# TuringLang/AdvancedHMC.jl

Measured on NVIDIA B200. Metric: leapfrog-steps*dims/sec, higher is better.
Workload: dtype f64

## Files before the change

### advancedhmc.jl_b200/__init__.py

```python
from . import _lib
from ._lib import (FLAG_ASYNC, FLAG_COMPAT_BREAK_ALL, FLAG_EXACT_CHECKS, FLAG_HOST_BUFFERS, FLAG_NO_REFRESH,
                   FLAG_NUTS_CLASSIC, FLAG_NUTS_SLICE_TS, FLAG_NUTS_STRICT,
                   STATUS_NONFINITE, AhmcError, InvalidArgument)
from .core import *
from .core import get_context
```

### advancedhmc.jl_b200/_lib.py

```python
from __future__ import annotations

import ctypes as C
import os

HERE = os.path.dirname(os.path.abspath(__file__))
LIB_PATH = os.environ.get("AHMC_B200_LIB", os.path.join(HERE, "libahmc_b200.so"))

OK, ERR_INVALID, ERR_CUDA, ERR_UNSUPPORTED, ERR_NOMEM, ERR_CALLBACK = 0, -1, -2, -3, -4, -5
METRIC_UNIT, METRIC_DIAG, METRIC_DENSE = 0, 1, 2
MODEL_STD_NORMAL, MODEL_DIAG_GAUSS, MODEL_DENSE_GAUSS, MODEL_FUNNEL, MODEL_CALLBACK, MODEL_USER = 0, 1, 2, 3, 4, 5
FLAG_HOST_BUFFERS, FLAG_COMPAT_BREAK_ALL, FLAG_ASYNC, FLAG_EXACT_CHECKS, FLAG_NO_REFRESH = 1, 2, 4, 8, 16
FLAG_NUTS_SLICE_TS, FLAG_NUTS_CLASSIC, FLAG_NUTS_STRICT = 32, 64, 128
STATUS_NONFINITE = 1

_dp = C.POINTER(C.c_double)
_vp = C.c_void_p


class Metric(C.Structure):
    _fields_ = [("kind", C.c_int32), ("Minv", _vp), ("chain_stride", C.c_int64), ("cholU", _vp)]


class PhasePoint(C.Structure):
    _fields_ = [("theta", _vp), ("r", _vp), ("lp_value", _vp), ("lp_gradient", _vp), ("lk_value", _vp),
                ("lk_gradient", _vp), ("ld", C.c_int64)]


class Stats(C.Structure):
    _fields_ = [("n_steps", _vp), ("is_accept", _vp), ("acceptance_rate", _vp), ("log_density", _vp),
                ("hamiltonian_energy", _vp), ("hamiltonian_energy_error", _vp),
                ("max_hamiltonian_energy_error", _vp), ("tree_depth", _vp), ("numerical_error", _vp)]


class Rng(C.Structure):
    _fields_ = [("seed", C.c_uint64), ("offset", C.c_uint64), ("normal_tape", _vp), ("exp_tape", _vp),
                ("exp_stride", C.c_int64), ("dir_tape", _vp), ("dir_stride", C.c_int64),
                ("partial_refresh_alpha", C.c_double), ("temper_alpha", C.c_double)]


class AdaptCfg(C.Structure):
    _fields_ = [("n_adapts", C.c_int32), ("init_buffer", C.c_int32), ("term_buffer", C.c_int32), ("window_size", C.c_int32),
                ("delta", C.c_double), ("gamma", C.c_double), ("t0", C.c_double), ("kappa", C.c_double),
                ("adapt_metric", C.c_int32), ("n_min", C.c_int32), ("eps_chain", _vp), ("Minv_chain", _vp),
                ("eps_trace", _vp)]


class PooledCfg(C.Structure):
    _fields_ = [("n_adapts", C.c_int32), ("init_buffer", C.c_int32), ("term_buffer", C.c_int32), ("window_size", C.c_int32),
                ("delta", C.c_double), ("gamma", C.c_double), ("t0", C.c_double), ("kappa", C.c_double), ("eps0", C.c_double),
                ("adapt_metric", C.c_int32), ("n_min", C.c_int32)]


LOGP_GRAD_FN = C.CFUNCTYPE(C.c_int, _vp, _vp, _vp, _vp, C.c_int32, C.c_int64, C.c_int64, _vp)

PROTOTYPES = {
    "ahmc_version": (C.c_char_p, []),
    "ahmc_create": (C.c_int, [C.POINTER(_vp), C.c_int32, _vp]),
    "ahmc_destroy": (C.c_int, [_vp]),
    "ahmc_last_error": (C.c_char_p, [_vp]),
    "ahmc_synchronize": (C.c_int, [_vp]),
    "ahmc_stream": (_vp, [_vp]),
    "ahmc_launch_count": (C.c_int64, [_vp]),
    "ahmc_last_transport": (C.c_char_p, [_vp]),
    "ahmc_model_create": (C.c_int, [_vp, C.c_int32, C.c_int32, _dp, _dp, C.c_double, C.POINTER(_vp)]),
    "ahmc_model_create_callback": (C.c_int, [_vp, C.c_int32, LOGP_GRAD_FN, _vp, C.POINTER(_vp)]),
    "ahmc_model_create_user": (C.c_int, [_vp, C.c_int32, C.c_char_p, _dp, C.c_int32, C.c_double, C.POINTER(_vp)]),
    "ahmc_user_source_check": (C.c_int, [C.c_char_p, C.c_int32, C.c_int32, C.c_int32, C.c_char_p, C.c_int64]),
    "ahmc_model_destroy": (C.c_int, [_vp, _vp]),
    "ahmc_phasepoint_f64": (C.c_int, [_vp, _vp, C.POINTER(Metric), C.c_int32, C.c_int64, C.POINTER(PhasePoint),
                                      C.c_uint32]),
    "ahmc_leapfrog_f64": (C.c_int, [_vp, _vp, C.POINTER(Metric), C.c_int32, C.c_int64, C.c_double, _vp, C.c_int32,
                                    C.c_double, C.POINTER(PhasePoint), C.POINTER(PhasePoint), _vp, _vp, C.c_uint32]),
    "ahmc_leapfrog_trajectory_f64": (C.c_int, [_vp, _vp, C.POINTER(Metric), C.c_int32, C.c_int64, C.c_double, _vp,
                                               C.c_int32, C.c_double, C.POINTER(PhasePoint), C.POINTER(PhasePoint),
                                               C.c_int64, _vp, C.c_uint32]),
    "ahmc_hmc_multinomial_transition_f64": (C.c_int, [_vp, _vp, C.POINTER(Metric), C.c_int32, C.c_int64, C.c_double, _vp,
                                                      C.c_int32, C.c_int32, C.POINTER(Rng), C.POINTER(PhasePoint),
                                                      C.POINTER(PhasePoint), C.POINTER(Stats), C.c_uint32]),
    "ahmc_rand_momentum_f64": (C.c_int, [_vp, C.POINTER(Metric), C.c_int32, C.c_int64, C.POINTER(Rng), _vp,
                                         C.c_int64, C.c_uint32]),
    "ahmc_hmc_transition_f64": (C.c_int, [_vp, _vp, C.POINTER(Metric), C.c_int32, C.c_int64, C.c_double, _vp,
                                          C.c_int32, C.POINTER(Rng), C.POINTER(PhasePoint), C.POINTER(PhasePoint),
                                          C.POINTER(Stats), C.c_uint32]),
    "ahmc_nuts_transition_f64": (C.c_int, [_vp, _vp, C.POINTER(Metric), C.c_int32, C.c_int64, C.c_double, _vp,
                                           C.c_int32, C.c_double, C.POINTER(Rng), C.POINTER(PhasePoint),
                                           C.POINTER(PhasePoint), C.POINTER(Stats), C.c_uint32]),
    "ahmc_hmc_sample_f64": (C.c_int, [_vp, _vp, C.POINTER(Metric), C.c_int32, C.c_int64, C.c_double, _vp, C.c_int32,
                                      C.c_int32, C.POINTER(Rng), C.POINTER(PhasePoint), C.POINTER(PhasePoint), _vp,
                                      C.POINTER(Stats), C.c_uint32]),
    "ahmc_nuts_sample_f64": (C.c_int, [_vp, _vp, C.POINTER(Metric), C.c_int32, C.c_int64, C.c_double, _vp, C.c_int32,
                                       C.c_double, C.c_int32, C.POINTER(Rng), C.POINTER(PhasePoint),
                                       C.POINTER(PhasePoint), _vp, C.POINTER(Stats), C.c_uint32]),
    "ahmc_nuts_adapt_sample_f64": (C.c_int, [_vp, _vp, C.POINTER(Metric), C.c_int32, C.c_int64, C.c_int32, C.c_double,
                                             C.c_int32, C.POINTER(AdaptCfg), C.POINTER(Rng), C.POINTER(PhasePoint),
                                             C.POINTER(PhasePoint), _vp, C.POINTER(Stats), C.c_uint32]),
# ... 46 lines not shown
```

### advancedhmc.jl_b200/csrc/ahmc_leapfrog.cu

```cuda
#ifndef __CUDACC_RTC__
#include <cstdlib>
#endif
#include "ahmc_kernels.cuh"
#include "ahmc_traj.cuh"

namespace ahmc {

bool pick_layout(int D, int* G, int* E) {
    if (D < 1) return false;
    if (D <= 4) { *G = 4; *E = 1; return true; }
    if (D <= 8) { *G = 8; *E = 1; return true; }
    if (D <= 16) { *G = 16; *E = 1; return true; }
    if (D <= 32) { *G = 32; *E = 1; return true; }
    if (D <= 64) { *G = 32; *E = 2; return true; }
    if (D <= 128) { *G = 32; *E = 4; return true; }
    if (D <= 256) { *G = 32; *E = 8; return true; }
    if (D <= 512) { *G = 32; *E = 16; return true; }
    return false;
}

template <int G, int E, bool CONTIG = false>
struct StepIO {
    static constexpr bool kContig = CONTIG;
    const LeapfrogArgs& a;
    long long chain;
    int l;
    __device__ __forceinline__ bool has_g() const { return a.g_in != nullptr; }
    __device__ __forceinline__ void init(double (&th)[E], double (&r)[E], double (&g)[E]) const {
        vload_nc<G, E>(th, a.th_in + a.ld_in * chain, l, a.D);
        vload_nc<G, E>(r, a.r_in + a.ld_in * chain, l, a.D);
        if (a.g_in) vload_nc<G, E>(g, a.g_in + a.ld_in * chain, l, a.D);
    }
    __device__ __forceinline__ void init_c(double (&th)[E], double (&r)[E], double (&g)[E]) const {
        cload<E>(th, a.th_in + a.ld_in * chain, l, a.D);
        cload<E>(r, a.r_in + a.ld_in * chain, l, a.D);
        cload<E>(g, (a.g_in ? a.g_in : a.th_in) + a.ld_in * chain, l, a.D);
    }
    __device__ __forceinline__ void scalars(double lp, double lk, bool fin, int steps) const {
        if (l == 0) {
            a.lp_out[chain] = lp;
            a.lk_out[chain] = lk;
            if (a.status) a.status[chain] = fin ? 0u : AHMC_STATUS_NONFINITE;
            if (a.steps_done) a.steps_done[chain] = steps;
            if (!fin && a.min_break) atomicMin(a.min_break, steps);
        }
    }
    __device__ __forceinline__ void done(const double (&th)[E], const double (&r)[E], const double (&g)[E],
                                         const double (&dr)[E], double lp, double lk, bool fin, int steps) const {
        vstore<G, E>(a.th_out + a.ld_out * chain, th, l, a.D);
        vstore<G, E>(a.r_out + a.ld_out * chain, r, l, a.D);
        vstore<G, E>(a.g_out + a.ld_out * chain, g, l, a.D);
        if (a.dr_out) vstore<G, E>(a.dr_out + a.ld_out * chain, dr, l, a.D);
        scalars(lp, lk, fin, steps);
    }
    __device__ __forceinline__ void done_c(const double (&th)[E], const double (&r)[E], const double (&g)[E],
                                           const double (&dr)[E], double lp, double lk, bool fin, int steps) const {
        cstore<E>(a.th_out + a.ld_out * chain, th, l, a.D);
        cstore<E>(a.r_out + a.ld_out * chain, r, l, a.D);
        cstore<E>(a.g_out + a.ld_out * chain, g, l, a.D);
        if (a.dr_out) cstore<E>(a.dr_out + a.ld_out * chain, dr, l, a.D);
        scalars(lp, lk, fin, steps);
    }
};

template <int MODEL, int METRIC, int E>
constexpr int min_blocks_per_sm() {
    return (FastCapable<MODEL, METRIC>::value && E <= 4) ? 7 : 1;
}
template <int MODEL, int METRIC, int E>
constexpr int min_blocks_hmc() {
    return (FastCapable<MODEL, METRIC>::value && E <= 4) ? 7 : ((METRIC != AHMC_METRIC_DENSE && MODEL != AHMC_MODEL_DENSE_GAUSS && E <= 4) ? 4 : 1);
}
template <int MODEL, int METRIC, int E>
constexpr int min_blocks_lf() {
    return (MODEL == AHMC_MODEL_FUNNEL && METRIC != AHMC_METRIC_DENSE && E <= 4) ? 7 : min_blocks_per_sm<MODEL, METRIC, E>();
}

template <int MODEL, int METRIC, int G, int E, bool CONTIG = false>
__global__ void __launch_bounds__(kBlockThreads, min_blocks_lf<MODEL, METRIC, E>()) leapfrog_kernel(const LeapfrogArgs a) {
    extern __shared__ double smem[];
    const int l = threadIdx.x % G;
    const int grp_in_block = threadIdx.x / G;
    const long long chain0 = (long long)blockIdx.x * (kBlockThreads / G) + grp_in_block;
    const long long chain = chain0 < a.N ? chain0 : a.N - 1;
    const bool valid = chain0 < a.N && (!a.only_mask || a.only_mask[chain] != 0);
    double* xs = smem + (size_t)grp_in_block * slab_vectors<MODEL>() * a.D;
    double eps = a.eps_chain ? __ldg(a.eps_chain + chain) : a.eps;
    eps = a.fwd ? eps : -eps;
    StepIO<G, E, CONTIG> io{a, chain, l};
    run_trajectory<MODEL, METRIC, G, E>(a.model, a.metric, a.D, chain, valid, l, xs, eps, a.n_steps, a.temper_alpha,
                                        a.flags, io);
}

template <int METRIC, int G, int E>
struct HmcIO {
    const HmcArgs& h;
    long long chain;
    int l;
    const double* src_th;
    const double* src_g;
    long long stat_idx;
    double H0, lp0, lk0, ex;
    double r0[E];

    static constexpr bool kContig = false;
    __device__ __forceinline__ bool has_g() const { return true; }
    __device__ __forceinline__ void init(double (&th)[E], double (&r)[E], double (&g)[E]) const {
        vload_nc<G, E>(th, src_th, l, h.lf.D);
        vload_nc<G, E>(g, src_g, l, h.lf.D);
#pragma unroll
        for (int e = 0; e < E; ++e) r[e] = r0[e];
    }
    __device__ __forceinline__ void done(const double (&th)[E], const double (&r)[E], const double (&g)[E],
                                         const double (&dr)[E], double lp, double lk, bool fin, int steps) const {
        const LeapfrogArgs& a = h.lf;
        const double H1 = -(lp + lk);
        const bool accept = H1 < H0 + ex;
        double alpha = exp(H0 - H1);
        alpha = (alpha != alpha) ? alpha : (alpha < 1.0 ? alpha : 1.0);
        double* tho = a.th_out + a.ld_out * chain;
        double* ro = a.r_out + a.ld_out * chain;
        double* go = a.g_out + a.ld_out * chain;
        double* dro = h.draws ? h.draws + stat_idx * a.D : nullptr;
        double lpn, lkn;
        if (accept) {
            double nr[E];
#pragma unroll
            for (int e = 0; e < E; ++e) nr[e] = -r[e];
            vstore<G, E>(tho, th, l, a.D);
            vstore<G, E>(ro, nr, l, a.D);
            vstore<G, E>(go, g, l, a.D);
            if (dro) vstore<G, E>(dro, th, l, a.D);
            lpn = lp;
            lkn = lk;
        } else {
            double t0[E], g0[E], nr[E];
            vload_nc<G, E>(t0, src_th, l, a.D);
            vload_nc<G, E>(g0, src_g, l, a.D);
#pragma unroll
            for (int e = 0; e < E; ++e) nr[e] = -r0[e];
            vstore<G, E>(tho, t0, l, a.D);
            vstore<G, E>(ro, nr, l, a.D);
            vstore<G, E>(go, g0, l, a.D);
            if (dro) vstore<G, E>(dro, t0, l, a.D);
            lpn = lp0;
            lkn = lk0;
        }
        if (l == 0) {
            const double H = -(lpn + lkn);
            a.lp_out[chain] = lpn;
            a.lk_out[chain] = lkn;
            if (a.status) a.status[chain] = fin ? 0u : AHMC_STATUS_NONFINITE;
            if (a.steps_done) a.steps_done[chain] = steps;
            const StatsDev& st = h.st;
            if (st.n_steps) st.n_steps[stat_idx] = a.n_steps;
            if (st.is_accept) st.is_accept[stat_idx] = accept ? 1 : 0;
            if (st.acceptance_rate) st.acceptance_rate[stat_idx] = alpha;
            if (st.log_density) st.log_density[stat_idx] = lpn;
            if (st.hamiltonian_energy) st.hamiltonian_energy[stat_idx] = H;
            if (st.hamiltonian_energy_error) st.hamiltonian_energy_error[stat_idx] = H - H0;
            if (st.numerical_error) st.numerical_error[stat_idx] = finite_d(H1) ? 0 : 1;
        }
        (void)dr;
    }
};

template <int MODEL, int METRIC, int G, int E>
__global__ void __launch_bounds__(kBlockThreads, min_blocks_hmc<MODEL, METRIC, E>()) hmc_kernel(const HmcArgs h) {
    extern __shared__ double smem[];
    const LeapfrogArgs& a = h.lf;
    const int l = threadIdx.x % G;
    const int grp_in_block = threadIdx.x / G;
    const long long chain0 = (long long)blockIdx.x * (kBlockThreads / G) + grp_in_block;
    const bool valid = chain0 < a.N;
// ... 214 lines not shown
    const double lp = a.cb_lp ? a.cb_lp[chain] : 0.0;
    bool fin = true;
#pragma unroll
    for (int e = 0; e < E; ++e) fin = fin && finite_d(g[e]) && finite_d(dr[e]);
    fin = Grp<G>::all(fin) && finite_d(lp) && finite_d(lk);
    if (active) {
        if (!a.no_kick) vstore<G, E>(a.r + a.ld * chain, r, l, D);
        if (a.cb_grad) vstore<G, E>(a.g + a.ld * chain, g, l, D);
        if (a.dr) vstore<G, E>(a.dr + a.ld * chain, dr, l, D);
        if (l == 0) {
            if (a.cb_lp) a.lp[chain] = map_nonfinite(lp);
            a.lk[chain] = map_nonfinite(lk);
            if (!a.no_kick) {
                if (a.steps_done) a.steps_done[chain] = a.step_index;
                if (!fin) {
                    a.status[chain] = AHMC_STATUS_NONFINITE;
                    if (a.any_nonfinite) *a.any_nonfinite = 1;
                }
            }
        }
    }
}

template <int G, int E>
__global__ void __launch_bounds__(kBlockThreads) mh_select_kernel(const MhArgs a) {
    const int l = threadIdx.x % G;
    const long long chain0 = (long long)blockIdx.x * (kBlockThreads / G) + threadIdx.x / G;
    if (chain0 >= a.N) return;
    const long long chain = chain0;
    const int D = a.D;
    const double lp0 = map_nonfinite(a.lp0[chain]), lk0 = a.lk0[chain];
    const double lp1 = a.lp[chain], lk1 = a.lk[chain];
    const double H0 = -(lp0 + lk0), H1 = -(lp1 + lk1);
    const double ex = a.rng.exp_tape ? a.rng.exp_tape[chain] : philox_exp(a.rng.seed, a.rng.offset, chain, 0);
    const bool accept = H1 < H0 + ex;
    double alpha = exp(H0 - H1);
    alpha = (alpha != alpha) ? alpha : (alpha < 1.0 ? alpha : 1.0);
    double t[E];
    if (accept) {
        vload_nc<G, E>(t, a.r + a.ld * chain, l, D);
#pragma unroll
        for (int e = 0; e < E; ++e) t[e] = -t[e];
        vstore<G, E>(a.r + a.ld * chain, t, l, D);
    } else {
        vload_nc<G, E>(t, a.th0 + a.ld0 * chain, l, D);
        vstore<G, E>(a.th + a.ld * chain, t, l, D);
        vload_nc<G, E>(t, a.g0 + a.ld0 * chain, l, D);
        vstore<G, E>(a.g + a.ld * chain, t, l, D);
        vload_nc<G, E>(t, a.r0 + (long long)D * chain, l, D);
#pragma unroll
        for (int e = 0; e < E; ++e) t[e] = -t[e];
        vstore<G, E>(a.r + a.ld * chain, t, l, D);
    }
    if (l == 0) {
        const double lpn = accept ? lp1 : lp0, lkn = accept ? lk1 : lk0;
        const double H = -(lpn + lkn);
        a.lp[chain] = lpn;
        a.lk[chain] = lkn;
        const StatsDev& st = a.st;
        if (st.n_steps) st.n_steps[chain] = a.n_steps;
        if (st.is_accept) st.is_accept[chain] = accept ? 1 : 0;
        if (st.acceptance_rate) st.acceptance_rate[chain] = alpha;
        if (st.log_density) st.log_density[chain] = lpn;
        if (st.hamiltonian_energy) st.hamiltonian_energy[chain] = H;
        if (st.hamiltonian_energy_error) st.hamiltonian_energy_error[chain] = H - H0;
        if (st.numerical_error) st.numerical_error[chain] = finite_d(H1) ? 0 : 1;
    }
}

#ifndef AHMC_SIMT_EMULATION
#ifndef __CUDACC_RTC__
template <int E>
static bool contig_ok(const LeapfrogArgs& a) {
    constexpr int V = E >= 4 ? 4 : E;
    const uintptr_t m = (uintptr_t)(8 * V - 1);
    auto al = [&](const void* p) { return ((uintptr_t)p & m) == 0; };
    if (a.D != 32 * E || a.ld_in % V || a.ld_out % V) return false;
    if (!al(a.th_in) || !al(a.r_in) || !al(a.g_in) || !al(a.th_out) || !al(a.r_out) || !al(a.g_out) || !al(a.dr_out)) return false;
    if (a.metric.kind == AHMC_METRIC_DIAG && (!al(a.metric.Minv) || a.metric.chain_stride % V)) return false;
    if (a.model.kind == AHMC_MODEL_DIAG_GAUSS && (!al(a.model.p0) || !al(a.model.p1))) return false;
    return true;
}

template <int MODEL, int METRIC, int G, int E, bool CONTIG>
static cudaError_t launch_lf_c(const LeapfrogArgs& a, cudaStream_t st) {
    const int chains_per_block = kBlockThreads / G;
    const long long blocks = (a.N + chains_per_block - 1) / chains_per_block;
    size_t sm = smem_bytes(MODEL, METRIC, a.D, G);
    const int occ = a.resident_blocks_per_sm;
    if (occ > 0) {
        const size_t pad = (size_t)(227 * 1024) / (size_t)occ - 1024;
        if (pad > sm) sm = pad;
    }
    if (sm > 48 * 1024) {
        cudaError_t e = cudaFuncSetAttribute(leapfrog_kernel<MODEL, METRIC, G, E, CONTIG>,
                                             cudaFuncAttributeMaxDynamicSharedMemorySize, (int)sm);
        if (e != cudaSuccess) return e;
    }
    leapfrog_kernel<MODEL, METRIC, G, E, CONTIG><<<(unsigned)blocks, kBlockThreads, sm, st>>>(a);
    return cudaGetLastError();
}
template <int MODEL, int METRIC, int G, int E>
static cudaError_t launch_lf_t(const LeapfrogArgs& a, cudaStream_t st) {
    if constexpr (FastCapable<MODEL, METRIC>::value && G == 32 && E >= 2) {
        if (!(a.flags & AHMC_FLAG_EXACT_CHECKS) && !(a.temper_alpha > 0.0) && contig_ok<E>(a))
            return launch_lf_c<MODEL, METRIC, G, E, true>(a, st);
    }
    return launch_lf_c<MODEL, METRIC, G, E, false>(a, st);
}
template <int MODEL, int METRIC, int G, int E>
static cudaError_t launch_fe_t(const FindEpsArgs& a, cudaStream_t st) {
    const int chains_per_block = kBlockThreads / G;
    const long long blocks = (a.N + chains_per_block - 1) / chains_per_block;
    size_t sm = smem_bytes(MODEL, METRIC, a.D, G);
    if (sm > 48 * 1024) {
        cudaError_t e = cudaFuncSetAttribute(find_eps_kernel<MODEL, METRIC, G, E>, cudaFuncAttributeMaxDynamicSharedMemorySize, (int)sm);
        if (e != cudaSuccess) return e;
    }
    find_eps_kernel<MODEL, METRIC, G, E><<<(unsigned)blocks, kBlockThreads, sm, st>>>(a);
    return cudaGetLastError();
}
template <int MODEL, int METRIC, int G, int E>
static cudaError_t launch_pp_t(const PhasepointArgs& a, cudaStream_t st) {
    const int chains_per_block = kBlockThreads / G;
    const long long blocks = (a.N + chains_per_block - 1) / chains_per_block;
    size_t sm = smem_bytes(MODEL, METRIC, a.D, G);
    if (sm > 48 * 1024) {
        cudaError_t e = cudaFuncSetAttribute(phasepoint_kernel<MODEL, METRIC, G, E>,
                                             cudaFuncAttributeMaxDynamicSharedMemorySize, (int)sm);
        if (e != cudaSuccess) return e;
    }
    phasepoint_kernel<MODEL, METRIC, G, E><<<(unsigned)blocks, kBlockThreads, sm, st>>>(a);
    return cudaGetLastError();
}
template <int MODEL, int METRIC, int G, int E>
static cudaError_t launch_hmc_t(const HmcArgs& a, cudaStream_t st) {
    const int chains_per_block = kBlockThreads / G;
    const long long blocks = (a.lf.N + chains_per_block - 1) / chains_per_block;
    size_t sm = smem_bytes(MODEL, METRIC, a.lf.D, G);
    if (sm > 48 * 1024) {
        cudaError_t e = cudaFuncSetAttribute(hmc_kernel<MODEL, METRIC, G, E>,
                                             cudaFuncAttributeMaxDynamicSharedMemorySize, (int)sm);
        if (e != cudaSuccess) return e;
    }
    hmc_kernel<MODEL, METRIC, G, E><<<(unsigned)blocks, kBlockThreads, sm, st>>>(a);
    return cudaGetLastError();
}
template <int METRIC, int G, int E>
static cudaError_t launch_kd_t(const SplitArgs& a, cudaStream_t st) {
    const long long blocks = (a.N + kBlockThreads / G - 1) / (kBlockThreads / G);
    size_t sm = smem_bytes(AHMC_MODEL_STD_NORMAL, METRIC, a.D, G);
    if (sm > 48 * 1024) {
        cudaError_t e = cudaFuncSetAttribute(kick_drift_kernel<METRIC, G, E>, cudaFuncAttributeMaxDynamicSharedMemorySize, (int)sm);
        if (e != cudaSuccess) return e;
    }
    kick_drift_kernel<METRIC, G, E><<<(unsigned)blocks, kBlockThreads, sm, st>>>(a);
    return cudaGetLastError();
}
template <int METRIC, int G, int E>
static cudaError_t launch_ke_t(const SplitArgs& a, cudaStream_t st) {
    const long long blocks = (a.N + kBlockThreads / G - 1) / (kBlockThreads / G);
    size_t sm = smem_bytes(AHMC_MODEL_STD_NORMAL, METRIC, a.D, G);
    if (sm > 48 * 1024) {
        cudaError_t e = cudaFuncSetAttribute(kick_energy_kernel<METRIC, G, E>, cudaFuncAttributeMaxDynamicSharedMemorySize, (int)sm);
        if (e != cudaSuccess) return e;
    }
    kick_energy_kernel<METRIC, G, E><<<(unsigned)blocks, kBlockThreads, sm, st>>>(a);
    return cudaGetLastError();
}
template <int DUMMY, int G, int E>
static cudaError_t launch_mh_t(const MhArgs& a, cudaStream_t st) {
    const long long blocks = (a.N + kBlockThreads / G - 1) / (kBlockThreads / G);
    mh_select_kernel<G, E><<<(unsigned)blocks, kBlockThreads, 0, st>>>(a);
    return cudaGetLastError();
}
template <int METRIC, int G, int E>
static cudaError_t launch_mom_t(const MomentumArgs& a, cudaStream_t st) {
    const int chains_per_block = kBlockThreads / G;
    const long long blocks = (a.N + chains_per_block - 1) / chains_per_block;
    momentum_kernel<METRIC, G, E><<<(unsigned)blocks, kBlockThreads, 0, st>>>(a);
    return cudaGetLastError();
}

#define AHMC_DISPATCH_LAYOUT(FN, ...)                                   \
    do {                                                                \
        if (G == 4 && E == 1) return FN<__VA_ARGS__, 4, 1>(a, st);      \
        if (G == 8 && E == 1) return FN<__VA_ARGS__, 8, 1>(a, st);      \
        if (G == 16 && E == 1) return FN<__VA_ARGS__, 16, 1>(a, st);    \
        if (G == 32 && E == 1) return FN<__VA_ARGS__, 32, 1>(a, st);    \
        if (G == 32 && E == 2) return FN<__VA_ARGS__, 32, 2>(a, st);    \
        if (G == 32 && E == 4) return FN<__VA_ARGS__, 32, 4>(a, st);    \
        if (G == 32 && E == 8) return FN<__VA_ARGS__, 32, 8>(a, st);    \
        if (G == 32 && E == 16) return FN<__VA_ARGS__, 32, 16>(a, st);  \
        return cudaErrorInvalidValue;                                   \
    } while (0)

template <int MODEL, int METRIC>
static cudaError_t lf_layout(const LeapfrogArgs& a, cudaStream_t st, int G, int E) {
    AHMC_DISPATCH_LAYOUT(launch_lf_t, MODEL, METRIC);
}
template <int MODEL, int METRIC>
static cudaError_t fe_layout(const FindEpsArgs& a, cudaStream_t st, int G, int E) {
    AHMC_DISPATCH_LAYOUT(launch_fe_t, MODEL, METRIC);
}
template <int MODEL, int METRIC>
static cudaError_t pp_layout(const PhasepointArgs& a, cudaStream_t st, int G, int E) {
    AHMC_DISPATCH_LAYOUT(launch_pp_t, MODEL, METRIC);
}
template <int MODEL, int METRIC>
static cudaError_t hmc_layout(const HmcArgs& a, cudaStream_t st, int G, int E) {
    AHMC_DISPATCH_LAYOUT(launch_hmc_t, MODEL, METRIC);
}
template <int METRIC>
static cudaError_t kd_layout(const SplitArgs& a, cudaStream_t st, int G, int E) {
    AHMC_DISPATCH_LAYOUT(launch_kd_t, METRIC);
}
template <int METRIC>
static cudaError_t ke_layout(const SplitArgs& a, cudaStream_t st, int G, int E) {
    AHMC_DISPATCH_LAYOUT(launch_ke_t, METRIC);
}
template <int DUMMY>
static cudaError_t mh_layout(const MhArgs& a, cudaStream_t st, int G, int E) {
    AHMC_DISPATCH_LAYOUT(launch_mh_t, DUMMY);
}
template <int METRIC>
static cudaError_t mom_layout(const MomentumArgs& a, cudaStream_t st, int G, int E) {
    AHMC_DISPATCH_LAYOUT(launch_mom_t, METRIC);
}

#define AHMC_DISPATCH_MM(FN, model_kind, metric_kind)                                                   \
    do {                                                                                                \
        switch ((model_kind) * 3 + (metric_kind)) {                                                     \
            case 0: return FN<AHMC_MODEL_STD_NORMAL, AHMC_METRIC_UNIT>(a, st, G, E);                    \
            case 1: return FN<AHMC_MODEL_STD_NORMAL, AHMC_METRIC_DIAG>(a, st, G, E);                    \
            case 2: return FN<AHMC_MODEL_STD_NORMAL, AHMC_METRIC_DENSE>(a, st, G, E);                   \
            case 3: return FN<AHMC_MODEL_DIAG_GAUSS, AHMC_METRIC_UNIT>(a, st, G, E);                    \
            case 4: return FN<AHMC_MODEL_DIAG_GAUSS, AHMC_METRIC_DIAG>(a, st, G, E);                    \
            case 5: return FN<AHMC_MODEL_DIAG_GAUSS, AHMC_METRIC_DENSE>(a, st, G, E);                   \
            case 6: return FN<AHMC_MODEL_DENSE_GAUSS, AHMC_METRIC_UNIT>(a, st, G, E);                   \
            case 7: return FN<AHMC_MODEL_DENSE_GAUSS, AHMC_METRIC_DIAG>(a, st, G, E);                   \
            case 8: return FN<AHMC_MODEL_DENSE_GAUSS, AHMC_METRIC_DENSE>(a, st, G, E);                  \
            case 9: return FN<AHMC_MODEL_FUNNEL, AHMC_METRIC_UNIT>(a, st, G, E);                        \
            case 10: return FN<AHMC_MODEL_FUNNEL, AHMC_METRIC_DIAG>(a, st, G, E);                       \
            case 11: return FN<AHMC_MODEL_FUNNEL, AHMC_METRIC_DENSE>(a, st, G, E);                      \
        }                                                                                               \
        return cudaErrorInvalidValue;                                                                   \
    } while (0)

cudaError_t launch_leapfrog(const LeapfrogArgs& a, cudaStream_t st, int* n_launches) {
    int G, E;
    if (a.D > 512) {
        if (n_launches) *n_launches += 1;
        return launch_leapfrog_big(a, st);
    }
    if (!pick_layout(a.D, &G, &E)) return cudaErrorInvalidValue;
    if (n_launches) *n_launches += 1;
    if (a.model.kind == AHMC_MODEL_USER) {
        const int cpb = kBlockThreads / G;
        return user_launch((UserModule*)a.model.user, UK_LEAPFROG, a.metric.kind, G, E, &a, (unsigned)((a.N + cpb - 1) / cpb),
                           smem_bytes(AHMC_MODEL_USER, a.metric.kind, a.D, G), st);
    }
    AHMC_DISPATCH_MM(lf_layout, a.model.kind, a.metric.kind);
}

cudaError_t launch_find_eps(const FindEpsArgs& a, cudaStream_t st, int* n_launches) {
    int G, E;
    if (!pick_layout(a.D, &G, &E)) return cudaErrorInvalidValue;
    if (n_launches) *n_launches += 1;
    if (a.model.kind == AHMC_MODEL_USER) {
        const int cpb = kBlockThreads / G;
        return user_launch((UserModule*)a.model.user, UK_FIND_EPS, a.metric.kind, G, E, &a, (unsigned)((a.N + cpb - 1) / cpb),
                           smem_bytes(AHMC_MODEL_USER, a.metric.kind, a.D, G), st);
    }
    AHMC_DISPATCH_MM(fe_layout, a.model.kind, a.metric.kind);
}

cudaError_t launch_phasepoint(const PhasepointArgs& a, cudaStream_t st, int* n_launches) {
    int G, E;
    if (a.D > 512) {
        if (n_launches) *n_launches += 1;
        return launch_phasepoint_big(a, st);
    }
    if (!pick_layout(a.D, &G, &E)) return cudaErrorInvalidValue;
    if (n_launches) *n_launches += 1;
    if (a.model.kind == AHMC_MODEL_USER) {
        const int cpb = kBlockThreads / G;
        return user_launch((UserModule*)a.model.user, UK_PHASEPOINT, a.metric.kind, G, E, &a, (unsigned)((a.N + cpb - 1) / cpb),
                           smem_bytes(AHMC_MODEL_USER, a.metric.kind, a.D, G), st);
    }
    AHMC_DISPATCH_MM(pp_layout, a.model.kind, a.metric.kind);
}

cudaError_t launch_hmc(const HmcArgs& a, cudaStream_t st, int* n_launches) {
    int G, E;
    if (!pick_layout(a.lf.D, &G, &E)) return cudaErrorInvalidValue;
    if (n_launches) *n_launches += 1;
    if (a.lf.model.kind == AHMC_MODEL_USER) {
        const int cpb = kBlockThreads / G;
        return user_launch((UserModule*)a.lf.model.user, UK_HMC, a.lf.metric.kind, G, E, &a, (unsigned)((a.lf.N + cpb - 1) / cpb),
                           smem_bytes(AHMC_MODEL_USER, a.lf.metric.kind, a.lf.D, G), st);
    }
    AHMC_DISPATCH_MM(hmc_layout, a.lf.model.kind, a.lf.metric.kind);
}

cudaError_t launch_kick_drift(const SplitArgs& a, cudaStream_t st, int* n_launches) {
    int G, E;
    if (!pick_layout(a.D, &G, &E)) return cudaErrorInvalidValue;
    if (n_launches) *n_launches += 1;
    switch (a.metric.kind) {
        case AHMC_METRIC_UNIT: return kd_layout<AHMC_METRIC_UNIT>(a, st, G, E);
        case AHMC_METRIC_DIAG: return kd_layout<AHMC_METRIC_DIAG>(a, st, G, E);
        case AHMC_METRIC_DENSE: return kd_layout<AHMC_METRIC_DENSE>(a, st, G, E);
    }
    return cudaErrorInvalidValue;
}
cudaError_t launch_kick_energy(const SplitArgs& a, cudaStream_t st, int* n_launches) {
    int G, E;
    if (!pick_layout(a.D, &G, &E)) return cudaErrorInvalidValue;
    if (n_launches) *n_launches += 1;
    switch (a.metric.kind) {
        case AHMC_METRIC_UNIT: return ke_layout<AHMC_METRIC_UNIT>(a, st, G, E);
        case AHMC_METRIC_DIAG: return ke_layout<AHMC_METRIC_DIAG>(a, st, G, E);
        case AHMC_METRIC_DENSE: return ke_layout<AHMC_METRIC_DENSE>(a, st, G, E);
    }
    return cudaErrorInvalidValue;
}
cudaError_t launch_mh_select(const MhArgs& a, cudaStream_t st, int* n_launches) {
    int G, E;
    if (!pick_layout(a.D, &G, &E)) return cudaErrorInvalidValue;
    if (n_launches) *n_launches += 1;
    return mh_layout<0>(a, st, G, E);
}

cudaError_t launch_rand_momentum(const MomentumArgs& a, cudaStream_t st, int* n_launches) {
    int G, E;
    if (!pick_layout(a.D, &G, &E)) return cudaErrorInvalidValue;
    if (n_launches) *n_launches += 1;
    switch (a.metric.kind) {
        case AHMC_METRIC_UNIT: return mom_layout<AHMC_METRIC_UNIT>(a, st, G, E);
        case AHMC_METRIC_DIAG: return mom_layout<AHMC_METRIC_DIAG>(a, st, G, E);
        case AHMC_METRIC_DENSE: return mom_layout<AHMC_METRIC_DENSE>(a, st, G, E);
    }
    return cudaErrorInvalidValue;
}

#endif

// ... 4 lines not shown
```

### advancedhmc.jl_b200/csrc/ahmc_microbench.cu

```cuda
#include <cuda_runtime.h>

#include <cstdio>

namespace {

template <int CHAINS>
__global__ void __launch_bounds__(256) dfma_kernel(double* sink, int iters, double a, double b) {
    double x[CHAINS];
#pragma unroll
    for (int j = 0; j < CHAINS; ++j) x[j] = 1e-3 * (threadIdx.x + 1) + j;
    for (int i = 0; i < iters; ++i) {
#pragma unroll
        for (int u = 0; u < 8; ++u) {
#pragma unroll
            for (int j = 0; j < CHAINS; ++j) x[j] = fma(x[j], a, b);
        }
    }
    double s = 0.0;
#pragma unroll
    for (int j = 0; j < CHAINS; ++j) s += x[j];
    if (s == 123456.789) sink[blockIdx.x * blockDim.x + threadIdx.x] = s;
}

}

extern "C" int ahmc_mb_dfma_peak(int device, int iters, int reps, double* tflops_out, double* ms_out) {
    if (cudaSetDevice(device) != cudaSuccess) return -1;
    cudaDeviceProp prop{};
    if (cudaGetDeviceProperties(&prop, device) != cudaSuccess) return -1;
    const int blocks = prop.multiProcessorCount * 8, threads = 256;
    constexpr int CH = 8;
    double* sink = nullptr;
    if (cudaMalloc(&sink, sizeof(double) * blocks * threads) != cudaSuccess) return -2;
    cudaEvent_t e0, e1;
    cudaEventCreate(&e0);
    cudaEventCreate(&e1);
    dfma_kernel<CH><<<blocks, threads>>>(sink, iters, 0.999999, 1e-7);
    double best = 1e30;
    for (int r = 0; r < reps; ++r) {
        cudaEventRecord(e0);
        dfma_kernel<CH><<<blocks, threads>>>(sink, iters, 0.999999, 1e-7);
        cudaEventRecord(e1);
        if (cudaEventSynchronize(e1) != cudaSuccess) return -3;
        float ms = 0.f;
        cudaEventElapsedTime(&ms, e0, e1);
        if (ms < best) best = ms;
    }
    cudaEventDestroy(e0);
    cudaEventDestroy(e1);
    cudaFree(sink);
    const double flop = 2.0 * (double)blocks * threads * CH * 8.0 * iters;
    if (tflops_out) *tflops_out = flop / (best * 1e-3) / 1e12;
    if (ms_out) *ms_out = best;
    return cudaGetLastError() == cudaSuccess ? 0 : -4;
}
```

### include/ahmc_b200.h

```cpp
#ifndef AHMC_B200_H
#define AHMC_B200_H

#ifndef __CUDACC_RTC__
#include <stdint.h>
#endif

#ifdef __cplusplus
extern "C" {
#endif

#define AHMC_OK 0
#define AHMC_ERR_INVALID (-1)
#define AHMC_ERR_CUDA (-2)
#define AHMC_ERR_UNSUPPORTED (-3)
#define AHMC_ERR_NOMEM (-4)
#define AHMC_ERR_CALLBACK (-5)

#define AHMC_METRIC_UNIT 0
#define AHMC_METRIC_DIAG 1
#define AHMC_METRIC_DENSE 2

#define AHMC_MODEL_STD_NORMAL 0
#define AHMC_MODEL_DIAG_GAUSS 1
#define AHMC_MODEL_DENSE_GAUSS 2
#define AHMC_MODEL_FUNNEL 3
#define AHMC_MODEL_CALLBACK 4
#define AHMC_MODEL_USER 5

#define AHMC_FLAG_HOST_BUFFERS 0x1u
#define AHMC_FLAG_COMPAT_BREAK_ALL 0x2u
#define AHMC_FLAG_ASYNC 0x4u
#define AHMC_FLAG_EXACT_CHECKS 0x8u
#define AHMC_FLAG_NO_REFRESH 0x10u
#define AHMC_FLAG_NUTS_SLICE_TS 0x20u
#define AHMC_FLAG_NUTS_CLASSIC 0x40u
#define AHMC_FLAG_NUTS_STRICT 0x80u

#define AHMC_STATUS_NONFINITE 0x1u

typedef struct ahmc_ctx ahmc_ctx;
typedef struct ahmc_model ahmc_model;

typedef struct ahmc_metric {
    int32_t kind;
    const double* Minv;
    int64_t chain_stride;
    const double* cholU;
} ahmc_metric;

typedef struct ahmc_phasepoint {
    double* theta;
    double* r;
    double* lp_value;
    double* lp_gradient;
    double* lk_value;
    double* lk_gradient;
    int64_t ld;
} ahmc_phasepoint;

typedef struct ahmc_stats {
    int32_t* n_steps;
    uint8_t* is_accept;
    double* acceptance_rate;
    double* log_density;
    double* hamiltonian_energy;
    double* hamiltonian_energy_error;
    double* max_hamiltonian_energy_error;
    int32_t* tree_depth;
    uint8_t* numerical_error;
} ahmc_stats;

typedef struct ahmc_rng {
    uint64_t seed;
    uint64_t offset;
    const double* normal_tape;
    const double* exp_tape;
    int64_t exp_stride;
    const uint8_t* dir_tape;
    int64_t dir_stride;
    double partial_refresh_alpha;
    double temper_alpha;
} ahmc_rng;

typedef int (*ahmc_logp_grad_fn)(void* user, const double* theta, double* lp, double* grad, int32_t D, int64_t N,
                                 int64_t ld, void* stream);

const char* ahmc_version(void);
int ahmc_create(ahmc_ctx** out, int32_t device, void* cuda_stream );
int ahmc_destroy(ahmc_ctx* ctx);
const char* ahmc_last_error(const ahmc_ctx* ctx);
int ahmc_synchronize(ahmc_ctx* ctx);
void* ahmc_stream(const ahmc_ctx* ctx);
int64_t ahmc_launch_count(const ahmc_ctx* ctx);
const char* ahmc_last_transport(const ahmc_ctx* ctx);

int ahmc_model_create(ahmc_ctx* ctx, int32_t kind, int32_t D, const double* p0, const double* p1, double c0,
                      ahmc_model** out);
int ahmc_model_create_callback(ahmc_ctx* ctx, int32_t D, ahmc_logp_grad_fn fn, void* user, ahmc_model** out);
int ahmc_model_create_user(ahmc_ctx* ctx, int32_t D, const char* cuda_src, const double* params, int32_t n_params, double c0,
                           ahmc_model** out);
int ahmc_user_source_check(const char* cuda_src, int32_t kernel, int32_t metric_kind, int32_t D, char* log, int64_t log_len);
int ahmc_model_destroy(ahmc_ctx* ctx, ahmc_model* model);

int ahmc_phasepoint_f64(ahmc_ctx* ctx, const ahmc_model* model, const ahmc_metric* metric, int32_t D, int64_t N,
                        const ahmc_phasepoint* z, uint32_t flags);

int ahmc_leapfrog_f64(ahmc_ctx* ctx, const ahmc_model* model, const ahmc_metric* metric, int32_t D, int64_t N,
                      double eps, const double* eps_chain, int32_t n_steps, double temper_alpha,
                      const ahmc_phasepoint* z_in, const ahmc_phasepoint* z_out, uint32_t* status,
                      int32_t* steps_done, uint32_t flags);

int ahmc_leapfrog_trajectory_f64(ahmc_ctx* ctx, const ahmc_model* model, const ahmc_metric* metric, int32_t D,
                                 int64_t N, double eps, const double* eps_chain, int32_t n_steps, double temper_alpha,
                                 const ahmc_phasepoint* z_in, const ahmc_phasepoint* traj, int64_t step_stride,
                                 int32_t* steps_done, uint32_t flags);

int ahmc_rand_momentum_f64(ahmc_ctx* ctx, const ahmc_metric* metric, int32_t D, int64_t N, const ahmc_rng* rng,
                           double* r, int64_t ld, uint32_t flags);

// ... 80 lines not shown
```

Baseline: 1346 billion.

## Add persistent warp-specialized leapfrog kernel with TMA bulk-copy staging pipeline

Adds a persistent streaming leapfrog kernel for E==4 contiguous fast paths. One producer warp per block issues bulk global-to-shared copies of theta, r and gradient into a 32-stage mbarrier ring, and 16 consumer warps run trajectories from the staged data. The grid is capped at the SM count, with chains split evenly across blocks. The goal is to overlap input loads with compute and avoid per-chain load latency, at the cost of large shared memory use and one block per SM. It also adds optional globaltimer and SM-id instrumentation, an opt-out flag, and an empty-launch microbenchmark.

```diff
diff --git a/advancedhmc.jl_b200/__init__.py b/advancedhmc.jl_b200/__init__.py
--- a/advancedhmc.jl_b200/__init__.py
+++ b/advancedhmc.jl_b200/__init__.py
@@ -1,5 +1,5 @@
 from . import _lib
-from ._lib import (FLAG_ASYNC, FLAG_COMPAT_BREAK_ALL, FLAG_EXACT_CHECKS, FLAG_HOST_BUFFERS, FLAG_NO_REFRESH,
+from ._lib import (FLAG_ASYNC, FLAG_COMPAT_BREAK_ALL, FLAG_EXACT_CHECKS, FLAG_HOST_BUFFERS, FLAG_K1_NO_STREAM, FLAG_NO_REFRESH,
                    FLAG_NUTS_CLASSIC, FLAG_NUTS_SLICE_TS, FLAG_NUTS_STRICT,
                    STATUS_NONFINITE, AhmcError, InvalidArgument)
 from .core import *
diff --git a/advancedhmc.jl_b200/_lib.py b/advancedhmc.jl_b200/_lib.py
--- a/advancedhmc.jl_b200/_lib.py
+++ b/advancedhmc.jl_b200/_lib.py
@@ -11,6 +11,7 @@
 MODEL_STD_NORMAL, MODEL_DIAG_GAUSS, MODEL_DENSE_GAUSS, MODEL_FUNNEL, MODEL_CALLBACK, MODEL_USER = 0, 1, 2, 3, 4, 5
 FLAG_HOST_BUFFERS, FLAG_COMPAT_BREAK_ALL, FLAG_ASYNC, FLAG_EXACT_CHECKS, FLAG_NO_REFRESH = 1, 2, 4, 8, 16
 FLAG_NUTS_SLICE_TS, FLAG_NUTS_CLASSIC, FLAG_NUTS_STRICT = 32, 64, 128
+FLAG_K1_NO_STREAM = 256
 STATUS_NONFINITE = 1
 
 _dp = C.POINTER(C.c_double)
diff --git a/advancedhmc.jl_b200/csrc/ahmc_leapfrog.cu b/advancedhmc.jl_b200/csrc/ahmc_leapfrog.cu
--- a/advancedhmc.jl_b200/csrc/ahmc_leapfrog.cu
+++ b/advancedhmc.jl_b200/csrc/ahmc_leapfrog.cu
@@ -19,7 +19,37 @@
     return false;
 }
 
-template <int G, int E, bool CONTIG = false>
+constexpr int kTimelineWords = 5;
+__device__ unsigned long long* k1_timeline;
+__device__ __forceinline__ unsigned long long stamp_after(unsigned long long dep) {
+#if defined(AHMC_SIMT_EMULATION)
+    (void)dep;
+    return 0;
+#else
+    unsigned long long t = 0;
+    asm volatile("{\n.reg .pred p;\nsetp.ne.u64 p, %1, 0x7ff8dead0000beef;\n@p mov.u64 %0, %%globaltimer;\n}" : "+l"(t) : "l"(dep));
+    return t;
+#endif
+}
+#if defined(AHMC_SIMT_EMULATION)
+inline unsigned long long dbits(double) { return 0; }
+#else
+__device__ __forceinline__ unsigned long long dbits(double x) { return (unsigned long long)__double_as_longlong(x); }
+#endif
+__device__ __forceinline__ void stamp(long long chain, int l, int i, unsigned long long t) {
+    if (l == 0) {
+        k1_timeline[chain * kTimelineWords + i] = t;
+#if !defined(AHMC_SIMT_EMULATION)
+        if (i == 0) {
+            unsigned sm;
+            asm volatile("mov.u32 %0, %%smid;" : "=r"(sm));
+            k1_timeline[chain * kTimelineWords + 4] = sm;
+        }
+#endif
+    }
+}
+
+template <int G, int E, bool CONTIG = false, bool TL = false>
 struct StepIO {
     static constexpr bool kContig = CONTIG;
     const LeapfrogArgs& a;
@@ -35,6 +65,7 @@
         cload<E>(th, a.th_in + a.ld_in * chain, l, a.D);
         cload<E>(r, a.r_in + a.ld_in * chain, l, a.D);
         cload<E>(g, (a.g_in ? a.g_in : a.th_in) + a.ld_in * chain, l, a.D);
+        if constexpr (TL) stamp(chain, l, 1, stamp_after(dbits(th[E - 1]) ^ dbits(r[E - 1]) ^ dbits(g[E - 1])));
     }
     __device__ __forceinline__ void scalars(double lp, double lk, bool fin, int steps) const {
         if (l == 0) {
@@ -55,11 +86,45 @@
     }
     __device__ __forceinline__ void done_c(const double (&th)[E], const double (&r)[E], const double (&g)[E],
                                            const double (&dr)[E], double lp, double lk, bool fin, int steps) const {
+        if constexpr (TL) stamp(chain, l, 2, stamp_after(dbits(th[0]) ^ dbits(r[0]) ^ dbits(lk)));
         cstore<E>(a.th_out + a.ld_out * chain, th, l, a.D);
         cstore<E>(a.r_out + a.ld_out * chain, r, l, a.D);
         cstore<E>(a.g_out + a.ld_out * chain, g, l, a.D);
         if (a.dr_out) cstore<E>(a.dr_out + a.ld_out * chain, dr, l, a.D);
         scalars(lp, lk, fin, steps);
+        if constexpr (TL) stamp(chain, l, 3, stamp_after(0));
+    }
+};
+
+template <int E, bool TL = false>
+struct StreamIO : StepIO<32, E, true, TL> {
+    const double* stage;
+    uint64_t* full;
+    uint64_t* empty;
+    uint32_t parity;
+    static __device__ __forceinline__ void sload(double (&x)[E], const double* s, int l) {
+        constexpr int V = Contig<E>::V;
+#pragma unroll
+        for (int b = 0; b < E / V; ++b) {
+#pragma unroll
+            for (int j = 0; j < V; j += 2) {
+                const double2 v = *reinterpret_cast<const double2*>(s + 32 * V * b + V * l + j);
+                x[V * b + j] = v.x;
+                x[V * b + j + 1] = v.y;
+            }
+        }
+    }
+    __device__ __forceinline__ void init_c(double (&th)[E], double (&r)[E], double (&g)[E]) const {
+        constexpr int D = 32 * E;
+        const int l = this->l;
+        if constexpr (TL) stamp(this->chain, l, 0, stamp_after(0));
+        mbar_wait(full, parity);
+        sload(th, stage, l);
+        sload(r, stage + D, l);
+        sload(g, stage + (this->has_g() ? 2 * D : 0), l);
+        __syncwarp();
+        if (l == 0) mbar_arrive(empty);
+        if constexpr (TL) stamp(this->chain, l, 1, stamp_after(dbits(th[E - 1]) ^ dbits(r[E - 1]) ^ dbits(g[E - 1])));
     }
 };
 
@@ -76,7 +141,7 @@
     return (MODEL == AHMC_MODEL_FUNNEL && METRIC != AHMC_METRIC_DENSE && E <= 4) ? 7 : min_blocks_per_sm<MODEL, METRIC, E>();
 }
 
-template <int MODEL, int METRIC, int G, int E, bool CONTIG = false>
+template <int MODEL, int METRIC, int G, int E, bool CONTIG = false, bool TL = false>
 __global__ void __launch_bounds__(kBlockThreads, min_blocks_lf<MODEL, METRIC, E>()) leapfrog_kernel(const LeapfrogArgs a) {
     extern __shared__ double smem[];
     const int l = threadIdx.x % G;
@@ -84,12 +149,61 @@
     const long long chain0 = (long long)blockIdx.x * (kBlockThreads / G) + grp_in_block;
     const long long chain = chain0 < a.N ? chain0 : a.N - 1;
     const bool valid = chain0 < a.N && (!a.only_mask || a.only_mask[chain] != 0);
+    if constexpr (TL) stamp(chain, l, 0, stamp_after(0));
     double* xs = smem + (size_t)grp_in_block * slab_vectors<MODEL>() * a.D;
     double eps = a.eps_chain ? __ldg(a.eps_chain + chain) : a.eps;
     eps = a.fwd ? eps : -eps;
-    StepIO<G, E, CONTIG> io{a, chain, l};
+    StepIO<G, E, CONTIG, TL> io{a, chain, l};
     run_trajectory<MODEL, METRIC, G, E>(a.model, a.metric, a.D, chain, valid, l, xs, eps, a.n_steps, a.temper_alpha,
                                         a.flags, io);
+}
+
+template <int E>
+__host__ __device__ constexpr size_t stream_smem_bytes(int S) { return (size_t)S * (3 * 32 * E * 8 + 2 * 8); }
+
+template <int MODEL, int METRIC, int E, int W, int S, bool TL = false>
+__global__ void __launch_bounds__(32 * (W + 1), 1) leapfrog_stream_kernel(const LeapfrogArgs a) {
+    extern __shared__ double smem[];
+    constexpr int D = 32 * E;
+    const int w = threadIdx.x >> 5, l = threadIdx.x & 31;
+    uint64_t* full = reinterpret_cast<uint64_t*>(smem + (size_t)S * 3 * D);
+    uint64_t* empty = full + S;
+    const long long per = a.N / gridDim.x, extra = a.N % gridDim.x;
+    const long long c0 = (long long)blockIdx.x * per + ((long long)blockIdx.x < extra ? blockIdx.x : extra);
+    const int cnt = (int)(per + ((long long)blockIdx.x < extra ? 1 : 0));
+    if (threadIdx.x == 0) {
+        for (int s = 0; s < S; ++s) {
+            mbar_init(&full[s], 1);
+            mbar_init(&empty[s], 1);
+        }
+        mbar_fence_init();
+    }
+    __syncthreads();
+    if (w == W) {
+        if (l == 0) {
+            constexpr uint32_t row = D * 8;
+            for (int k = 0; k < cnt; ++k) {
+                const int s = k % S;
+                if (k >= S) mbar_wait(&empty[s], (uint32_t)((k / S - 1) & 1));
+                double* st = smem + (size_t)s * 3 * D;
+                const long long off = a.ld_in * (c0 + k);
+                mbar_expect_tx(&full[s], a.g_in ? 3 * row : 2 * row);
+                bulk_g2s(st, a.th_in + off, row, &full[s]);
+                bulk_g2s(st + D, a.r_in + off, row, &full[s]);
+                if (a.g_in) bulk_g2s(st + 2 * D, a.g_in + off, row, &full[s]);
+            }
+        }
+        return;
+    }
+    for (int k = w; k < cnt; k += W) {
+        const long long chain = c0 + k;
+        double eps = a.eps_chain ? __ldg(a.eps_chain + chain) : a.eps;
+        eps = a.fwd ? eps : -eps;
+        const int s = k % S;
+        StreamIO<E, TL> io{{a, chain, l}, smem + (size_t)s * 3 * D, &full[s], &empty[s], (uint32_t)((k / S) & 1)};
+        run_trajectory<MODEL, METRIC, 32, E>(a.model, a.metric, D, chain, true, l, smem, eps, a.n_steps, a.temper_alpha,
+                                             a.flags, io);
+    }
 }
 
 template <int METRIC, int G, int E>
@@ -470,7 +584,9 @@
     return true;
 }
 
-template <int MODEL, int METRIC, int G, int E, bool CONTIG>
+static unsigned long long* g_timeline_host = nullptr;
+
+template <int MODEL, int METRIC, int G, int E, bool CONTIG, bool TL>
 static cudaError_t launch_lf_c(const LeapfrogArgs& a, cudaStream_t st) {
     const int chains_per_block = kBlockThreads / G;
     const long long blocks = (a.N + chains_per_block - 1) / chains_per_block;
@@ -481,20 +597,51 @@
         if (pad > sm) sm = pad;
     }
     if (sm > 48 * 1024) {
-        cudaError_t e = cudaFuncSetAttribute(leapfrog_kernel<MODEL, METRIC, G, E, CONTIG>,
+        cudaError_t e = cudaFuncSetAttribute(leapfrog_kernel<MODEL, METRIC, G, E, CONTIG, TL>,
                                              cudaFuncAttributeMaxDynamicSharedMemorySize, (int)sm);
         if (e != cudaSuccess) return e;
     }
-    leapfrog_kernel<MODEL, METRIC, G, E, CONTIG><<<(unsigned)blocks, kBlockThreads, sm, st>>>(a);
+    leapfrog_kernel<MODEL, METRIC, G, E, CONTIG, TL><<<(unsigned)blocks, kBlockThreads, sm, st>>>(a);
+    return cudaGetLastError();
+}
+
+constexpr int kStreamWarps = 16, kStreamStages = 32;
+
+static int sm_count() {
+    int dev = 0, n = 0;
+    if (cudaGetDevice(&dev) != cudaSuccess || cudaDeviceGetAttribute(&n, cudaDevAttrMultiProcessorCount, dev) != cudaSuccess) return 0;
+    return n;
+}
+
+template <int MODEL, int METRIC, int E, bool TL>
+static cudaError_t launch_lf_stream(const LeapfrogArgs& a, cudaStream_t st) {
+    constexpr int W = kStreamWarps, S = kStreamStages;
+    const size_t sm = stream_smem_bytes<E>(S);
+    const int n_sm = sm_count();
+    if (n_sm <= 0) return cudaErrorInvalidDevice;
+    if (sm > 48 * 1024) {
+        cudaError_t e = cudaFuncSetAttribute(leapfrog_stream_kernel<MODEL, METRIC, E, W, S, TL>,
+                                             cudaFuncAttributeMaxDynamicSharedMemorySize, (int)sm);
+        if (e != cudaSuccess) return e;
+    }
+    const long long blocks = a.N < n_sm ? a.N : n_sm;
+    leapfrog_stream_kernel<MODEL, METRIC, E, W, S, TL><<<(unsigned)blocks, 32 * (W + 1), sm, st>>>(a);
     return cudaGetLastError();
 }
 template <int MODEL, int METRIC, int G, int E>
 static cudaError_t launch_lf_t(const LeapfrogArgs& a, cudaStream_t st) {
     if constexpr (FastCapable<MODEL, METRIC>::value && G == 32 && E >= 2) {
-        if (!(a.flags & AHMC_FLAG_EXACT_CHECKS) && !(a.temper_alpha > 0.0) && contig_ok<E>(a))
-            return launch_lf_c<MODEL, METRIC, G, E, true>(a, st);
-    }
-    return launch_lf_c<MODEL, METRIC, G, E, false>(a, st);
+        if (!(a.flags & AHMC_FLAG_EXACT_CHECKS) && !(a.temper_alpha > 0.0) && contig_ok<E>(a)) {
+            constexpr bool kTL = MODEL == AHMC_MODEL_DIAG_GAUSS && METRIC == AHMC_METRIC_DIAG && E == 4;
+            const bool tl = kTL && g_timeline_host != nullptr;
+            if constexpr (E == 4) {
+                if (!(a.flags & AHMC_FLAG_K1_NO_STREAM) && a.resident_blocks_per_sm == 0 && !a.only_mask)
+                    return tl ? launch_lf_stream<MODEL, METRIC, E, kTL>(a, st) : launch_lf_stream<MODEL, METRIC, E, false>(a, st);
+            }
+            return tl ? launch_lf_c<MODEL, METRIC, G, E, true, kTL>(a, st) : launch_lf_c<MODEL, METRIC, G, E, true, false>(a, st);
+        }
+    }
+    return launch_lf_c<MODEL, METRIC, G, E, false, false>(a, st);
 }
 template <int MODEL, int METRIC, int G, int E>
 static cudaError_t launch_fe_t(const FindEpsArgs& a, cudaStream_t st) {
@@ -651,6 +798,12 @@
     AHMC_DISPATCH_MM(lf_layout, a.model.kind, a.metric.kind);
 }
 
+extern "C" int ahmc_internal_k1_timeline(unsigned long long* stamps) {
+    if (cudaMemcpyToSymbol(k1_timeline, &stamps, sizeof(stamps)) != cudaSuccess) return AHMC_ERR_CUDA;
+    g_timeline_host = stamps;
+    return 0;
+}
+
 cudaError_t launch_find_eps(const FindEpsArgs& a, cudaStream_t st, int* n_launches) {
     int G, E;
     if (!pick_layout(a.D, &G, &E)) return cudaErrorInvalidValue;
diff --git a/advancedhmc.jl_b200/csrc/ahmc_microbench.cu b/advancedhmc.jl_b200/csrc/ahmc_microbench.cu
--- a/advancedhmc.jl_b200/csrc/ahmc_microbench.cu
+++ b/advancedhmc.jl_b200/csrc/ahmc_microbench.cu
@@ -2,7 +2,14 @@
 
 #include <cstdio>
 
+#include "ahmc_kernels.cuh"
+
 namespace {
+
+struct K1Params {
+    unsigned char bytes[sizeof(ahmc::LeapfrogArgs)];
+};
+__global__ void empty_kernel(const K1Params) {}
 
 template <int CHAINS>
 __global__ void __launch_bounds__(256) dfma_kernel(double* sink, int iters, double a, double b) {
@@ -54,3 +61,10 @@
     if (ms_out) *ms_out = best;
     return cudaGetLastError() == cudaSuccess ? 0 : -4;
 }
+
+extern "C" int ahmc_mb_empty_launch(unsigned grid, unsigned block, unsigned smem, void* stream) {
+    if (smem > 48 * 1024 && cudaFuncSetAttribute(empty_kernel, cudaFuncAttributeMaxDynamicSharedMemorySize, (int)smem) != cudaSuccess)
+        return -1;
+    empty_kernel<<<grid, block, smem, (cudaStream_t)stream>>>(K1Params{});
+    return cudaGetLastError() == cudaSuccess ? 0 : -2;
+}
diff --git a/include/ahmc_b200.h b/include/ahmc_b200.h
--- a/include/ahmc_b200.h
+++ b/include/ahmc_b200.h
@@ -35,6 +35,7 @@
 #define AHMC_FLAG_NUTS_SLICE_TS 0x20u
 #define AHMC_FLAG_NUTS_CLASSIC 0x40u
 #define AHMC_FLAG_NUTS_STRICT 0x80u
+#define AHMC_FLAG_K1_NO_STREAM 0x100u
 
 #define AHMC_STATUS_NONFINITE 0x1u
 
```

Result: slower. 1198 billion (median of 6 runs) (-11.0%).
